# evandez/neuron-descriptions

Hardware: AMD Instinct MI355X
Metric: neuron-descriptions/sec (whole node), 4096 neurons x k=15 exemplars (higher is better)
Workload: dtype f32-equivalent: operands split into (hi,lo) f16 pairs (22 significant bits), 3 f16 MFMAs per product, f32 accumulate

## Files before the change

### neuron-descriptions_amd/csrc/common.h

```cpp
#pragma once
#include <hip/hip_runtime.h>
#include <stdint.h>
#include <stddef.h>
#include <string>
#include <vector>
#include <map>

#include "../../include/milan_hip.h"

#ifndef MILAN_EXPERIMENTS
#define MILAN_EXPERIMENTS 0
#endif

namespace milan {

void set_error(const char* fmt, ...);
#define MILAN_CHECK_HIP(expr)                                              \
  do {                                                                     \
    hipError_t _e = (expr);                                                \
    if (_e != hipSuccess) {                                                \
      milan::set_error("%s:%d: %s -> %s", __FILE__, __LINE__, #expr,       \
                       hipGetErrorString(_e));                             \
      return (int)_e;                                                      \
    }                                                                      \
// ... 54 lines not shown
  int chunk_major;
  float* C2;
  float* Cs;
  unsigned* status;
  int f16;
  const float* Wt;
  int tap_inner;
  const long long* lse_tgt;
  long lse_tgt_stride;
  float* lse_x;
  const int* m_live;
  const int* row_list;
  int m_live_mul;
  int tap_ncls;
  int tap_cls[MILAN_TAP_CLASSES][5];
};
static_assert(sizeof(GemmArgs) % 4 == 0, "GemmArgs is reloaded word by word");

enum OutMode : int { OUT_SCALAR = 0, OUT_VEC4 = 1, OUT_SPLIT8 = 2, OUT_F16 = 3 };

int launch_gemm(const GemmArgs& g, hipStream_t s);
bool row_list_supported(const GemmArgs& g);
void set_status_word(unsigned* word);
unsigned* status_word();
void profile_tag_kernel(int family);
int launch_zero_fill(void* p, size_t bytes, hipStream_t s);
int launch_f32_to_split(const float* src, long ld_src, float* dst, long ld_dst,
                        long rows, int K, float scale, hipStream_t s, int* nanrow = nullptr,
                        int stamp = 0);
int gemm_profile_enable(int enable);
int ensure_lds_attr(const void* kern, int bytes);
int device_cus8(int* out);
void* gemm_profile_begin(double flops, double bytes, hipStream_t s);
void gemm_profile_end(void* rec, hipStream_t s);

struct ShareArgs {
  const unsigned char* images;
// ... 410 lines not shown
```

### neuron-descriptions_amd/csrc/decoder.hip

```cpp
#include "common.h"
#include <limits>
#include <optional>

namespace milan {

static constexpr float kFloatMin = -3.402823466e+38f;

static const Tensor* find(milan_ctx* c, const std::string& name) {
  auto it = c->raw.find(name);
  return it == c->raw.end() ? nullptr : &it->second;
}

__global__ void pack_rows_kernel(const float* __restrict__ src, int n, int k,
                                 int kp, float* __restrict__ dst) {
  const long total = (long)n * kp;
  for (long idx = blockIdx.x * (long)blockDim.x + threadIdx.x; idx < total;
       idx += (long)gridDim.x * blockDim.x) {
    const int r = idx / kp, col = idx - (long)r * kp;
    dst[idx] = col < k ? src[(long)r * k + col] : 0.f;
  }
}

__device__ inline int lstm_source_row(int i, int hidden) {
  if (!hidden) return i;
// ... 157 lines not shown
    const int f = idx - i * F;
    float s = 0.f;
    for (int j = 0; j < k; ++j) {
      const float x = feat[(i * k + j) * F + f];
      sat = fmaxf(sat, fabsf(x * scale));
      s += x;
    }
    pooled[idx] = s / (float)k;
  }
  report_saturation(status, sat);
}

__global__ __launch_bounds__(256) void attend_kernel(
    const float* __restrict__ q, const float* __restrict__ keys,
    const float* __restrict__ w, const float* __restrict__ b, int rows, int rpn,
    int k, int A, float* __restrict__ att, const int* __restrict__ nanrow, int stamp) {
  const int r = blockIdx.x * 4 + (threadIdx.x >> 6);
  const int lane = threadIdx.x & 63;
  if (r >= rows) return;
  const float* qr = q + (long)r * A;
  const float* kr = keys + (long)(r / rpn) * k * A;
  float mine = 0.f;
  float mx = -INFINITY;
  for (int j = 0; j < k; ++j) {
    float s = 0.f;
    for (int a = lane; a < A; a += 64) s += w[a] * tanhf(qr[a] + kr[(long)j * A + a]);
    for (int o = 32; o > 0; o >>= 1) s += __shfl_xor(s, o);
    s += b[0];
    if (lane == (j & 63)) mine = s;
    mx = fmaxf(mx, s);
  }
  float e = lane < k ? expf(mine - mx) : 0.f;
  float sum = e;
  for (int o = 32; o > 0; o >>= 1) sum += __shfl_xor(sum, o);
  const bool bad = nanrow != nullptr && nanrow[r] == stamp;
  if (lane < k) att[(long)r * k + lane] = bad ? __builtin_nanf("") : e / sum;
}

constexpr int kAttMaxK = 16, kAttMaxE = 8;
__device__ __forceinline__ float tanh_exp2(float x) {
  const float t = __builtin_amdgcn_exp2f(x * 2.8853900817779268f);
  return 1.f - 2.f * __builtin_amdgcn_rcpf(t + 1.f);
}
__global__ __launch_bounds__(256) void attend16_kernel(
    const float* __restrict__ q, const float* __restrict__ keys,
    const float* __restrict__ w, const float* __restrict__ b, int rows, int rpn,
    int k, int A, float* __restrict__ att, const int* __restrict__ nanrow, int stamp) {
  const int neuron = blockIdx.x;
  const int wave = blockIdx.y * 4 + (threadIdx.x >> 6), lane = threadIdx.x & 63;
  const int stride = 4 * gridDim.y;
  const int r0 = neuron * rpn;
  const int r1 = r0 + rpn < rows ? r0 + rpn : rows;
  if (r0 + wave >= r1) return;
  const float* kr = keys + (long)neuron * k * A;
  const int ne = (A + 63) / 64;
  float wv[kAttMaxE], kv[kAttMaxK][kAttMaxE];
  int av[kAttMaxE];
#pragma unroll
  for (int e = 0; e < kAttMaxE; ++e) {
    const int a = lane + 64 * e;
    const bool ok = a < A;
    av[e] = ok ? a : 0;
    wv[e] = ok ? w[a] : 0.f;
  }
#pragma unroll
  for (int j = 0; j < kAttMaxK; ++j)
#pragma unroll
// ... 33 lines not shown
    float mx = valid ? s : -INFINITY;
#pragma unroll
    for (int X = 4; X < 64; X <<= 1) mx = fmaxf(mx, __shfl_xor(mx, X));
    const bool writer = valid && (lane & 3) == 0;
    const float ev = writer ? expf(s - mx) : 0.f;
    float sum = ev;
#pragma unroll
    for (int X = 4; X < 64; X <<= 1) sum += __shfl_xor(sum, X);
    const bool bad = nanrow != nullptr && nanrow[r] == stamp;
    if (writer) att[(long)r * k + j] = bad ? __builtin_nanf("") : ev / sum;
  }
}

static void launch_attend(const float* q, const float* keys, const float* w, const float* b,
                          int rows, int rpn, int k, int A, float* att, const int* nanrow,
                          int stamp, hipStream_t s) {
  static const bool fast = !(getenv("MILAN_ATTEND_FAST") && atoi(getenv("MILAN_ATTEND_FAST")) == 0);
  if (fast && k <= kAttMaxK && A <= 64 * kAttMaxE) {
    const int neurons = (rows + rpn - 1) / rpn;
    int rs = (4096 + neurons * 4 - 1) / (neurons * 4);
    const int rs_max = (rpn + 3) / 4;
    rs = rs < 1 ? 1 : (rs > rs_max ? rs_max : rs);
    hipLaunchKernelGGL(attend16_kernel, dim3(neurons, rs), dim3(256), 0, s, q, keys, w, b, rows,
                       rpn, k, A, att, nanrow, stamp);
  } else {
    hipLaunchKernelGGL(attend_kernel, dim3((rows + 3) / 4), dim3(256), 0, s, q, keys, w, b,
                       rows, rpn, k, A, att, nanrow, stamp);
  }
}

constexpr int kCtxMaxK = 16;
template <bool RESIDENT>
__global__ __launch_bounds__(256) void context_kernel(
    const float* __restrict__ att, const float* __restrict__ feat, int rows,
    int rpn, int k, int F, float* __restrict__ ctx, float scale,
    int* __restrict__ nanrow, int stamp) {
  const int neuron = blockIdx.x;
  const int f = (blockIdx.y * 256 + threadIdx.x) * 4;
  if (f >= F) return;
  const float* fr = feat + (long)neuron * k * F + f;
  float4 v[RESIDENT ? kCtxMaxK : 1];
  if constexpr (RESIDENT) {
#pragma unroll
    for (int j = 0; j < kCtxMaxK; ++j)
      v[j] = j < k ? *reinterpret_cast<const float4*>(fr + (long)j * F)
                   : make_float4(0.f, 0.f, 0.f, 0.f);
  }
  const int r0 = neuron * rpn;
  const int r1 = r0 + rpn < rows ? r0 + rpn : rows;
  for (int r = r0; r < r1; ++r) {
    const float* ar = att + (long)r * k;
    float s0 = 0.f, s1 = 0.f, s2 = 0.f, s3 = 0.f;
    if constexpr (RESIDENT) {
#pragma unroll
      for (int j = 0; j < kCtxMaxK; ++j) {
        if (j < k) {
          const float aj = ar[j];
          s0 = fmaf(aj, v[j].x, s0); s1 = fmaf(aj, v[j].y, s1);
          s2 = fmaf(aj, v[j].z, s2); s3 = fmaf(aj, v[j].w, s3);
        }
      }
    } else {
      for (int j = 0; j < k; ++j) {
        const float4 w = *reinterpret_cast<const float4*>(fr + (long)j * F);
// ... 17 lines not shown
                             float* __restrict__ dst, int ldd, float scale) {
  const long total = (long)rows * E;
  for (long idx = blockIdx.x * (long)blockDim.x + threadIdx.x; idx < total;
       idx += (long)gridDim.x * blockDim.x) {
    const long r = idx / E;
    const int e = idx - r * E;
    dst[r * ldd + e] = table[tok[r] * E + e] * scale;
  }
}

__global__ void embed_split_kernel(const float* __restrict__ table,
                                   const int64_t* __restrict__ tok, int rows, int E,
                                   float* __restrict__ dst, int ldd, float scale,
                                   unsigned* status,
                                   const int* __restrict__ live = nullptr,
                                   const int* __restrict__ nanrow = nullptr, int stamp = 0) {
  if (live) rows = min(rows, *live);
  const int g8 = E >> 3;
  const long total = (long)rows * g8;
  float sat = 0.f;
  for (long idx = blockIdx.x * (long)blockDim.x + threadIdx.x; idx < total;
       idx += (long)gridDim.x * blockDim.x) {
    const long r = idx / g8;
    const int q = idx - r * g8;
    const float* sp = table + tok[r] * E + q * 8;
    _Float16 hi[8], lo[8];
#pragma unroll
    for (int e = 0; e < 8; ++e) {
      const float x = fminf(fmaxf(sp[e] * scale, -65504.f), 65504.f);
      sat = fmaxf(sat, fabsf(x));
      hi[e] = (_Float16)x;
      lo[e] = (_Float16)(x - (float)hi[e]);
    }
    if (nanrow != nullptr && nanrow[r] == stamp) {
#pragma unroll
      for (int e = 0; e < 8; ++e) hi[e] = (_Float16)__builtin_nanf("");
    }
    float4* d = reinterpret_cast<float4*>(dst + r * ldd + q * 8);
    d[0] = *reinterpret_cast<const float4*>(hi);
    d[1] = *reinterpret_cast<const float4*>(lo);
  }
  report_saturation(status, sat);
}

__global__ void lstm_pointwise_kernel(const float* __restrict__ gates,
                                      const float* __restrict__ c_in, int rows,
                                      int H, float* __restrict__ h_out,
                                      float* __restrict__ c_out) {
  const long total = (long)rows * H;
// ... 580 lines not shown
  }
}

__global__ void beam_reorder_kernel(
    const int* __restrict__ new_tok, const int* __restrict__ new_bp, int n,
    int beam_prev, int beam, int H, const float* __restrict__ h_src,
    const float* __restrict__ c_src, float* __restrict__ h_dst,
    float* __restrict__ c_dst, int lm_layers, int Hl, long lm_rows_src,
    long lm_rows_dst, const float* __restrict__ hl_src,
    const float* __restrict__ cl_src, float* __restrict__ hl_dst,
    float* __restrict__ cl_dst, int64_t* __restrict__ tok_dst,
    int* __restrict__ hist_tok, int* __restrict__ hist_bp) {
  const int r = blockIdx.x;
  const int nn = r / beam;
  const int src = nn * beam_prev + new_bp[r];
  for (int j = threadIdx.x; j < H; j += blockDim.x) {
    h_dst[(long)r * H + j] = h_src[(long)src * H + j];
    c_dst[(long)r * H + j] = c_src[(long)src * H + j];
  }
  for (int l = 0; l < lm_layers; ++l)
    for (int j = threadIdx.x; j < Hl; j += blockDim.x) {
      hl_dst[((long)l * lm_rows_dst + r) * Hl + j] =
          hl_src[((long)l * lm_rows_src + src) * Hl + j];
      cl_dst[((long)l * lm_rows_dst + r) * Hl + j] =
          cl_src[((long)l * lm_rows_src + src) * Hl + j];
    }
  if (threadIdx.x == 0) {
    tok_dst[r] = new_tok[r];
    hist_tok[r] = new_tok[r];
    hist_bp[r] = new_bp[r];
  }
}

__global__ void beam_finalize_kernel(const int* __restrict__ hist_tok,
                                     const int* __restrict__ hist_bp, int n,
                                     int beam, int T,
                                     int64_t* __restrict__ beam_tokens) {
  const int r = blockIdx.x * blockDim.x + threadIdx.x;
  if (r >= n * beam) return;
  const int nn = r / beam;
  int j = r - nn * beam;
  const long R = (long)n * beam;
  for (int t = T - 1; t >= 0; --t) {
    beam_tokens[(long)r * T + t] = hist_tok[t * R + nn * beam + j];
    j = hist_bp[t * R + nn * beam + j];
  }
// ... 256 lines not shown

struct DecBuf {
  float *keys, *pooled, *x, *h, *cc, *hn, *cn, *q, *att, *ctx, *gates, *logits;
  float *lm_logits, *lm_emb, *lm_gates;
  LmState lm[2];
  float* cand_v; int* cand_i;
  float* last_lp[2]; int *new_tok, *new_bp, *hist_tok, *hist_bp;
  int64_t *tok, *seqs;
  float *lm_alive, *lm_total;
  float* lm_dedup; size_t lm_dedup_floats;
  int32_t* len1;
  float* scratch;
  size_t scratch_floats;
  int* nanrow;
  int nan_stamp;
};

static size_t lm_dedup_floats(const milan_dims& d, size_t R, int L, int G);

static void dec_plan(const milan_ctx* c, int n, int k, int beam, int T, bool lm,
                     Arena& a, DecBuf* b) {
  const milan_dims& d = c->d;
  const size_t R = (size_t)n * beam;
  const int F = d.feature_size, H = d.hidden_size, E = d.embedding_size,
            A = d.attention_size, V = d.vocab_size;
  b->keys = a.get<float>((size_t)n * k * A);
  b->pooled = a.get<float>((size_t)n * F);
  b->x = a.get<float>(R * (E + F));
  b->h = a.get<float>(R * H); b->cc = a.get<float>(R * H);
  b->hn = a.get<float>(R * H); b->cn = a.get<float>(R * H);
  b->q = a.get<float>(R * A);
  b->att = a.get<float>(R * k);
  b->ctx = a.get<float>(R * F);
  b->gates = a.get<float>(R * 4 * H);
  b->logits = a.get<float>(R * V);
  b->cand_v = a.get<float>(R * beam); b->cand_i = a.get<int>(R * beam);
  b->last_lp[0] = a.get<float>(R); b->last_lp[1] = a.get<float>(R);
  b->new_tok = a.get<int>(R); b->new_bp = a.get<int>(R);
  b->hist_tok = a.get<int>(R * T); b->hist_bp = a.get<int>(R * T);
  b->tok = a.get<int64_t>(R);
  b->seqs = a.get<int64_t>(R * (T + 1));
  b->len1 = a.get<int32_t>(2 * (size_t)n + 2);
  b->nanrow = a.get<int>(R);
  b->nan_stamp = 0;
  {
    const size_t rows = R > (size_t)n * k ? R : (size_t)n * k;
    b->scratch_floats = rows * (size_t)(E + F + d.hidden_size);
    b->scratch = a.get<float>(b->scratch_floats);
  }
  b->lm_logits = nullptr;
  b->lm_dedup = nullptr; b->lm_dedup_floats = 0;
  if (lm) {
    const int Hl = d.lm_hidden_size, El = d.lm_embedding_size;
    b->lm_logits = a.get<float>(R * V);
    b->lm_emb = a.get<float>(R * El);
    b->lm_gates = a.get<float>(R * 4 * Hl);
    for (int i = 0; i < 2; ++i) {
      b->lm[i].h = a.get<float>(R * Hl * d.lm_layers);
      b->lm[i].c = a.get<float>(R * Hl * d.lm_layers);
// ... 45 lines not shown
  return 0;
}

int decoder_init_state(milan_ctx* c, const float* features, int n, int k,
                       float* h, float* cc, Arena& ws, hipStream_t s) {
  MILAN_TRY(check_dims(c, k));
  float* pooled = ws.get<float>((size_t)n * c->d.feature_size);
  MILAN_REQUIRE(pooled, MILAN_ERR_WORKSPACE, "init_state: workspace too small");
  c->scratch_floats = (size_t)n * c->d.feature_size;
  c->scratch = ws.get<float>(c->scratch_floats);
  return init_state_impl(c, features, n, k, pooled, h, cc, s);
}

static void launch_context(const float* att, const float* features, int rows,
                           int rpn, int k, int F, float* ctx, float scale,
                           int* nanrow, int stamp, hipStream_t s) {
  const int gy = (F / 4 + 255) / 256;
  const int neurons = (rows + rpn - 1) / rpn;
  if (k <= kCtxMaxK)
    hipLaunchKernelGGL(context_kernel<true>, dim3(neurons, gy), dim3(256), 0, s,
                       att, features, rows, rpn, k, F, ctx, scale, nanrow, stamp);
  else
    hipLaunchKernelGGL(context_kernel<false>, dim3(neurons, gy), dim3(256), 0, s,
                       att, features, rows, rpn, k, F, ctx, scale, nanrow, stamp);
}

static int step_core(milan_ctx* c, const float* features, const float* keys,
                     int rows, int rpn, int k, const int64_t* tok,
                     const float* h, const float* cc, float* hn, float* cn,
                     DecBuf* b, hipStream_t s) {
  const milan_dims& d = c->d;
  const int F = d.feature_size, H = d.hidden_size, E = d.embedding_size,
            A = d.attention_size, V = d.vocab_size;
  const int ldx = E + F;
  const bool fused = c->precision == MILAN_PRECISION_SPLIT_F16 && c->scratch &&
                     c->q2h.ws && c->gate.ws && c->lstm_cat.ws && c->out.ws &&
                     E % 16 == 0 && F % 8 == 0 && H % 16 == 0 &&
                     (size_t)rows * (ldx + H) <= c->scratch_floats;
  const bool cat_split = c->precision == MILAN_PRECISION_SPLIT_F16 && c->lstm_cat.ws &&
                         c->scratch && (size_t)rows * c->lstm_cat.k <= c->scratch_floats;
  const float fs = cat_split ? c->feat_scale : 1.f;
  if (fused) {
    float* xs = c->scratch;
    float* hs = c->scratch + (size_t)rows * ldx;
    float* hs2 = b->gates;
    const int stamp = ++b->nan_stamp;
    MILAN_TRY(launch_f32_to_split(h, H, hs, H, rows, H, 1.f, s, b->nanrow, stamp));
    auto split_lin = [&](const LinearW& w, float* C, int ldc, int epi,
                         const float* aux, int ldaux) {
      GemmArgs g = linear_args(hs, H, w.ws, w.b, C, ldc, rows, w.n, w.k, epi,
                               c->zero, aux, ldaux);
      g.a_split = 1;
      g.acc_scale = w.ws_inv;
      return g;
    };
    MILAN_TRY(launch_gemm(split_lin(c->q2h, b->q, A, EPI_BIAS, nullptr, 0), s));
// ... 554 lines not shown
                "row select: rows=%d, k=%d must be in 1..min(%d, vocab_size %d)", rows, k,
                kMaxBeam, V);
  if (path == 0)
    return launch_row_select(logits, lm_logits, lambda, rows, V, k, last_tok, stop,
                             cand_v, cand_i, nullptr, 0, s);
  if (path == 1)
    return launch_row_select_wide(logits, lm_logits, lambda, rows, V, k, last_tok, stop,
                                  cand_v, cand_i, s);
  MILAN_REQUIRE(k >= 2 && row_select_reg_ok(V, k), MILAN_ERR_ARG,
                "row select: path %d needs 2 <= k <= 256 and vocab_size <= %d (k=%d, "
                "vocab_size %d)", path, kRowRegs * 256, k, V);
  return launch_row_select(logits, lm_logits, lambda, rows, V, k, last_tok, stop, cand_v,
                           cand_i, nullptr, 0, s, false, path == 2 ? 0 : 2);
}

int decoder_decode(milan_ctx* c, const float* features, int n, int k,
                   int strategy, int length, int beam, int mi, float temperature,
                   int group_size, int64_t* tokens, float* scores,
                   float* predictions, float* attentions, int64_t* beam_tokens,
                   float* beam_scores, int32_t* out_len, Arena& ws,
                   hipStream_t s) {
  MILAN_TRY(check_dims(c, k));
  const milan_dims& d = c->d;
  const int H = d.hidden_size, V = d.vocab_size;
  MILAN_REQUIRE(strategy == MILAN_GREEDY || strategy == MILAN_FORCED ||
                    strategy == MILAN_BEAM || strategy == MILAN_RERANK,
                MILAN_ERR_ARG, "unknown strategy: %d", strategy);
  MILAN_REQUIRE(!(mi && strategy == MILAN_RERANK), MILAN_ERR_ARG,
                "cannot set `mi=` decoding when reranking");
  MILAN_REQUIRE(!(mi || strategy == MILAN_RERANK) || d.has_lm, MILAN_ERR_NO_LM,
// ... 68 lines not shown
                           predictions + (long)t * V, (long)length * V, V, b.att,
                           n, k, t, length, tokens, scores, attentions, b.tok);
      else
        hipLaunchKernelGGL(greedy_record_kernel, dim3(nblk_all(n)), dim3(256), 0, s,
                           b.cand_v, b.cand_i, b.att, n, k, t, length, tokens,
                           scores, attentions, b.tok);
      float* tmp = h; h = hn; hn = tmp;
      tmp = cc; cc = cn; cn = tmp;
    }
    MILAN_CHECK_HIP(hipGetLastError());
    return 0;
  }

  const bool wide = c->beam_path == 1;
  int beam_prev = 1, rows = n, lpcur = 0;
  std::optional<StageScope> search_scope;
  search_scope.emplace(MILAN_STAGE_DEC_SEARCH, s);
  for (int t = 0; t < length; ++t) {
    MILAN_TRY(step_core(c, features, b.keys, rows, beam_prev, k, b.tok, b.h, b.cc,
                        b.hn, b.cn, &b, s));
    const float* lm_logits = nullptr;
    if (mi) {
      b.lm[lmcur].rows = b.lm[lmcur ^ 1].rows = R;
      MILAN_TRY(lm_step(c, b.tok, rows, b.lm[lmcur], b.lm[lmcur ^ 1], b.lm_emb,
                        b.lm_gates, b.lm_logits, s));
      lm_logits = b.lm_logits;
    }
    MILAN_TRY(launch_row_select(b.logits, lm_logits, temperature, rows, V, beam,
                                t == 0 ? nullptr : b.tok, d.stop_index, b.cand_v,
                                b.cand_i, nullptr, 0, s, wide));
    MILAN_TRY(decoder_beam_merge(b.cand_v, b.cand_i, t == 0 ? nullptr : b.last_lp[lpcur],
                                 n, beam_prev, beam, wide, b.last_lp[lpcur ^ 1], b.new_tok,
                                 b.new_bp, s));
    lpcur ^= 1;
    hipLaunchKernelGGL(
        beam_reorder_kernel, dim3(R), dim3(128), 0, s, b.new_tok, b.new_bp, n,
        beam_prev, beam, H, b.hn, b.cn, b.h, b.cc, mi ? d.lm_layers : 0, Hl,
        (long)R, (long)R, mi ? b.lm[lmcur ^ 1].h : nullptr,
        mi ? b.lm[lmcur ^ 1].c : nullptr, mi ? b.lm[lmcur].h : nullptr,
        mi ? b.lm[lmcur].c : nullptr, b.tok, b.hist_tok + (long)t * R,
        b.hist_bp + (long)t * R);
    beam_prev = beam;
    rows = R;
  }
  hipLaunchKernelGGL(beam_finalize_kernel, dim3(nblk_all(R)), dim3(256), 0, s,
                     b.hist_tok, b.hist_bp, n, beam, length, beam_tokens);
  MILAN_CHECK_HIP(hipMemcpyAsync(beam_scores, b.last_lp[lpcur],
                                 sizeof(float) * R, hipMemcpyDeviceToDevice, s));
  const int groups = (n + group_size - 1) / group_size;
  int32_t* lens = out_len ? out_len : b.len1 + n + 1;
  hipLaunchKernelGGL(group_len_kernel, dim3(groups), dim3(256), 0, s, b.hist_tok,
                     n, beam, length, group_size, d.stop_index, lens);
// ... 23 lines not shown
```

### neuron-descriptions_amd/csrc/gemm.hip

```cpp
#include "common.h"

#include <map>
#include <mutex>
#include <utility>

#include <cstdio>
#include <cstdlib>
#include <cstring>
#include <type_traits>
#include <utility>
#include <vector>

#ifndef MILAN_ABLATE_BUILD
#define MILAN_ABLATE_BUILD 0
#endif
#ifndef MILAN_EXPERIMENTS
#define MILAN_EXPERIMENTS 0
#endif

namespace milan {

typedef float f32x16 __attribute__((ext_vector_type(16)));
typedef float f32x4 __attribute__((ext_vector_type(4)));
typedef _Float16 f16x8 __attribute__((ext_vector_type(8)));
// ... 1482 lines not shown
    if (cls < 0 && b < first + B) { cls = c; cfirst = first; ctiles = T; }
    first += B;
  }
  if (cls < 0) return false;
  const int bl = b - cfirst;
  if ((bl >> 3) >= (ctiles >> 3) + ((bl & 7) < (ctiles & 7))) return false;
  const int tile = xcd_tile(bl, ctiles);
  t->j = tile / tiles_n;
  t->tile_n = tile - t->j * tiles_n;
  t->y0 = cw[cls * 5]; t->ny = cw[cls * 5 + 1]; t->x0 = cw[cls * 5 + 2]; t->nx = cw[cls * 5 + 3];
  t->mask = (unsigned)cw[cls * 5 + 4];
  t->cnt = imgs * t->ny * t->nx;
  return true;
}

template <int BNW, bool F16 = false, bool TAPI = false, bool LIST = false>
__device__ __forceinline__ void split16_pp32_tile(int tile_m, int tile_n, int tid, bool prefetched,
                                                  bool has_next, int ntile_m, int ntile_n,
                                                  TapTile tt = TapTile{}) {
  const GemmArgs g = reload_gemm_args();
  constexpr int BM = 256, BN = 256, BKP = 32, TM = BNW == 256 ? 4 : 2, TN = 2;
  static_assert(BNW == 256 || BNW == 128, "ping-pong tile: 256 or 128 columns");
  constexpr int SLOTF = BM * BKP;
  constexpr unsigned OOB = 0x80000000u;
  extern __shared__ __attribute__((aligned(16))) float smem[];
  auto a_slot = [&](int sl) { return smem + (sl < 2 ? sl : 3) * SLOTF; };
  auto w_slot = [&](int sl) { return smem + (sl == 0 ? 2 : 4) * SLOTF; };
  const int lane = tid & 63;
  const int wave = __builtin_amdgcn_readfirstlane(tid >> 6);
  const int wm = BNW == 256 ? wave >> 2 : wave >> 1, wn = BNW == 256 ? wave & 3 : wave & 1;
  const int group = wave >> 2;
// ... 40 lines not shown
    ho += ((ho + 1) * pix_row <= rem);
    *dimg_out = dimg;
    *wo_out = rem - ho * pix_row + (TAPI ? tt.x0 : 0);
    *ho_out = ho + (TAPI ? tt.y0 : 0);
    return ok;
  };
  auto setup = [&](PpLoader& L, int tm, int tn) {
    const int prow = lane >> 3, pos = lane & 7;
    const int m0 = tm * BM;
    const int img0 = LIST ? list_slot0(m0) : m0 / pix_img;
    const int rem0 = LIST ? img0 * pix_img : m0 - img0 * pix_img;
    const long bias = ((long)g.pad * g.Wd + g.pad) * g.a_pix_stride;
    L.srd_a = __builtin_amdgcn_make_buffer_rsrc(
        const_cast<float*>(g.A + (long)img0 * g.a_img_stride - bias), 0, 0x7fffffff, 0x00020000);
    L.srd_a2 = __builtin_amdgcn_make_buffer_rsrc(
        const_cast<float*>(g.A2 ? g.A2 + (long)img0 * g.a2_img_stride : g.A), 0, 0x7fffffff,
        0x00020000);
    L.srd_w = __builtin_amdgcn_make_buffer_rsrc(const_cast<float*>(g.W + (long)tn * BNW * g.Kp), 0,
                                                0x7fffffff, 0x00020000);
#pragma unroll
    for (int it = 0; it < 4; ++it) {
      const int row = it * 64 + wave * 8 + prow;
      const int q = pos ^ ((row >> 1) & 7);
      int dimg, ho, wo;
      const bool ok = row_pixel(m0, rem0, row, &dimg, &ho, &wo);
      const int hi0 = ho * g.stride - g.pad, wi0 = wo * g.stride - g.pad;
      L.hw0[it] = (hi0 << 16) | (wi0 & 0xffff);
      if constexpr (TAPI) {
        unsigned m = 0;
        for (int kh = 0, t = 0; kh < g.KH; ++kh)
          for (int kw = 0; kw < g.KW; ++kw, ++t)
            m |= (unsigned)((unsigned)(hi0 + kh) < (unsigned)g.H &&
                            (unsigned)(wi0 + kw) < (unsigned)g.Wd) << t;
        L.mask[it] = m;
      }
      L.row_off[it] = ok ? (unsigned)(((long)dimg * g.a_img_stride +
                                       ((long)hi0 * g.Wd + wi0) * g.a_pix_stride + bias + q * 4) * 4)
                         : OOB;
      L.row_off2[it] = (ok && g.A2)
                           ? (unsigned)(((long)dimg * g.a2_img_stride +
                                         ((long)(ho * g.stride2) * g.W2d + wo * g.stride2) *
                                             g.a2_pix_stride + q * 4) * 4)
                           : OOB;
      L.vb[it] = (row < BNW && tn * BNW + row < g.N) ? (unsigned)(((long)row * g.Kp + q * 4) * 4) : OOB;
    }
    L.ia = L.iw = L.is_kh = L.is_kw = L.is_cin0 = 0;
    L.a_bits = L.w_bits = tt.mask;
    L.w_slice = 0;
    L.cin_limit = g.Cin;
    L.cur_srd = L.srd_a;
    set_tap(L);
  };
  auto issue_a = [&](PpLoader& L, auto slot_tag, bool really) {
    constexpr int SLOT = decltype(slot_tag)::value;
    if (really) {
      int woff = wave * (8 * BKP);
      asm volatile("" : "+s"(woff));
      float* dst = a_slot(SLOT) + woff;
// ... 322 lines not shown
  const int q = blockIdx.x;
  if (q >= T) return;
  const int tile = xcd_tile(q, T);
  const int tile_m = tile / tiles_n, tile_n = tile - tile_m * tiles_n;
  TapTile tt{};
  if constexpr (TAPI) {
    tt.ny = g.Ho; tt.nx = g.Wo;
    tt.mask = 0xffffffffu >> (32 - g.KH * g.KW);
    tt.cnt = g.M;
  }
  int tid = threadIdx.x;
  asm volatile("" : "+v"(tid));
  split16_pp32_tile<256, false, TAPI, true>(tile_m, tile_n, tid, false, false, tile_m, tile_n, tt);
}

template <int BNW, bool TAPI>
__global__ __launch_bounds__(512, 2) void igemm_f16_pp32_kernel(GemmArgs g, int tiles_m, int tiles_n) {
  tiles_m = live_tiles_m(g, tiles_m, 256);
  if constexpr (TAPI) {
    TapTile tt;
    if (!tap_tile(g, tiles_m, tiles_n, &tt)) return;
    int tid = threadIdx.x;
    asm volatile("" : "+v"(tid));
    split16_pp32_tile<BNW, true, true>(tt.j, tt.tile_n, tid, false, false, tt.j, tt.tile_n, tt);
  } else {
    const int T = tiles_m * tiles_n;
    const int q = blockIdx.x;
    if (q >= T) return;
    const int tile = xcd_tile(q, T);
    const int tile_m = tile / tiles_n, tile_n = tile - tile_m * tiles_n;
// ... 548 lines not shown
      memcpy(cls[at], c, sizeof(c));
      if (ry[a].n * rx[b].n < min_pix) min_pix = ry[a].n * rx[b].n;
    }
  if ((256L / min_pix + 2) * t.a_img_stride * 4 + 64 >= 0x7fffffffL) return tiles_m * tiles_n;
  const long imgs = t.M / howo;
  long grid = 0;
  for (int c = 0; c < n; ++c)
    grid += ((imgs * cls[c][1] * cls[c][3] + 255) / 256 * tiles_n + 7) / 8 * 8;
  if (grid >= 0x7fffffffL) return tiles_m * tiles_n;
  t.tap_ncls = n;
  memcpy(t.tap_cls, cls, sizeof(int) * 5 * n);
  return (int)grid;
}

static thread_local bool t_row_list_taken = false;

template <int BNW>
static int launch_split16_pp32(const GemmArgs& g, hipStream_t s) {
  const int tiles_m = (g.M + 255) / 256, tiles_n = (g.N + BNW - 1) / BNW;
  const size_t lds = size_t(5) * 256 * 32 * sizeof(float);
  if (g.row_list != nullptr) {
    if (BNW != 256) return MILAN_ERR_SHAPE;
    t_row_list_taken = true;
    GemmArgs t = g;
    const bool tapi = tap_inner_wanted(g);
    if (tapi) { t.W = g.Wt; t.tap_inner = 1; }
    t.tap_ncls = 0;
    profile_tag_kernel(tapi ? MILAN_KERNEL_PP32T_256 : MILAN_KERNEL_PP32_256);
    auto kern = tapi ? igemm_split16_pp32l_kernel<true> : igemm_split16_pp32l_kernel<false>;
    MILAN_TRY(ensure_lds_attr(reinterpret_cast<const void*>(kern), (int)lds));
    hipLaunchKernelGGL(kern, dim3(tiles_m * tiles_n), dim3(512), lds, s, t, tiles_m, tiles_n);
    MILAN_CHECK_HIP(hipGetLastError());
    return 0;
  }
  if (tap_inner_wanted(g)) {
    GemmArgs t = g;
    t.W = g.Wt;
    t.tap_inner = 1;
    const int grid = tap_classes(t, tiles_m, tiles_n);
    profile_tag_kernel(BNW == 256 ? MILAN_KERNEL_PP32T_256 : MILAN_KERNEL_PP32_128);
    auto kern = igemm_split16_pp32t_kernel<BNW>;
    MILAN_TRY(ensure_lds_attr(reinterpret_cast<const void*>(kern), (int)lds));
    hipLaunchKernelGGL(kern, dim3(grid), dim3(512), lds, s, t, tiles_m, tiles_n);
    MILAN_CHECK_HIP(hipGetLastError());
    return 0;
  }
// ... 174 lines not shown
  if (!g.a_split || g.f16 || g.chunk_major || g.aniso || g.tile_hint != 0 || env_tile_hint() != 0 ||
      env_tile_override(g.N, g.K) != 0 || pp != 1)
    return false;
#if MILAN_EXPERIMENTS
  if (conv3x3_enabled() || (getenv("MILAN_SCHED") && atoi(getenv("MILAN_SCHED")))) return false;
#endif
  if (g.epilogue == EPI_LSE || g.epilogue == EPI_LSTM || !g.out_split) return false;
  if (g.N % 256 != 0 || g.Cin % 32 != 0 || g.K != g.Kp || !pp_eligible(g)) return false;
  if (g.A2 && (g.K1 % 32 != 0 || g.KH != 1 || g.KW != 1)) return false;
  if (g.KH * g.KW > 1 && !tap_inner_wanted(g)) return false;
  if ((long)g.H + g.pad >= 32768 || (long)g.Wd + g.pad >= 32768) return false;
  if (howo <= 0 || g.M % howo != 0 || 257 * howo >= (1L << 24)) return false;
  if (258 * g.a_img_stride * 4 + 64 >= 0x7fffffffL) return false;
  if (g.A2 && 258 * g.a2_img_stride * 4 + 64 >= 0x7fffffffL) return false;
  return true;
}

static int launch_gemm_impl(GemmArgs g, hipStream_t s) {
  const bool cin32 = (g.Cin % 32 == 0);
  if (g.status == nullptr) g.status = status_word();
  if (g.tile_hint == 0) g.tile_hint = env_tile_hint();
  if (const int o = env_tile_override(g.N, g.K)) g.tile_hint = o;
  {
    static int dbg = -1;
    if (dbg < 0) { const char* e = getenv("MILAN_ABLATE"); dbg = e ? atoi(e) : 0; }
    g.debug = dbg;
#if MILAN_EXPERIMENTS
    static int stg = -1;
    if (stg < 0) { const char* e = getenv("MILAN_STAGGER"); stg = e ? atoi(e) : 0; }
    static int stg_all = -1;
// ... 110 lines not shown
               : launch_cfg<128, 128, 2, false, false>(g, s);
}

static int launch_gemm_checked(const GemmArgs& g, hipStream_t s);
int launch_gemm(const GemmArgs& g, hipStream_t s) {
  MILAN_REQUIRE(g.M > 0 && g.N > 0 && g.K > 0, MILAN_ERR_SHAPE,
                "gemm: empty problem M=%d N=%d K=%d", g.M, g.N, g.K);
  MILAN_REQUIRE(g.row_list == nullptr || row_list_supported(g), MILAN_ERR_SHAPE,
                "gemm: no row-list form of this launch (N=%d Cin=%d %dx%d)", g.N, g.Cin, g.KH, g.KW);
  MILAN_REQUIRE(g.Cin % 4 == 0 && g.a_pix_stride % 4 == 0 &&
                    g.a_img_stride % 4 == 0 && g.Kp % 32 == 0 && aligned16(g.A) &&
                    aligned16(g.W),
                MILAN_ERR_SHAPE,
                "gemm: Cin=%d / strides must be multiples of 4 floats and "
                "operands 16-byte aligned", g.Cin);
  if (g.row_list != nullptr) {
    t_row_list_taken = false;
    const int r = launch_gemm_checked(g, s);
    MILAN_REQUIRE(r != 0 || t_row_list_taken, MILAN_ERR_STATE,
                  "gemm: a row-list launch was dispatched to a kernel without a list form "
                  "(row_list_supported() no longer matches the dispatch)");
    return r;
  }
  return launch_gemm_checked(g, s);
}

static int launch_gemm_checked(const GemmArgs& g, hipStream_t s) {
  if (!g_prof.on) return launch_gemm_impl(g, s);
  ProfRec* e = prof_next();
  MILAN_REQUIRE(e != nullptr, MILAN_ERR_STATE, "profiler: cannot create events");
// ... 15 lines not shown
```

Measured before the change: 1425.

## Share parent-dependent decoder work across beams with identical back-pointers

During beam search, rows whose back-pointer names the same parent have identical hidden states for the attention query, attention, context and gate computations. New kernels build per-neuron parent classes (dedup, scan, fill), and the step runs q2h, attention, context and gate only on the unique parent rows. The LSTM GEMM then gathers its second operand through a row table (new A2TAB kernel variant), and the reorder kernel skips copying h. This cuts redundant GEMM and attention work when beams share parents, at the cost of extra small launches and an indirect row load in the GEMM.

Result: no change. 1437 (median of 5 runs) (+0.8%).

```diff
diff --git a/neuron-descriptions_amd/csrc/common.h b/neuron-descriptions_amd/csrc/common.h
--- a/neuron-descriptions_amd/csrc/common.h
+++ b/neuron-descriptions_amd/csrc/common.h
@@ -92,6 +92,7 @@
   int m_live_mul;
   int tap_ncls;
   int tap_cls[MILAN_TAP_CLASSES][5];
+  const int* a2_rows;
 };
 static_assert(sizeof(GemmArgs) % 4 == 0, "GemmArgs is reloaded word by word");
 
@@ -99,6 +100,7 @@
 
 int launch_gemm(const GemmArgs& g, hipStream_t s);
 bool row_list_supported(const GemmArgs& g);
+bool a2_rows_supported(const GemmArgs& g);
 void set_status_word(unsigned* word);
 unsigned* status_word();
 void profile_tag_kernel(int family);
diff --git a/neuron-descriptions_amd/csrc/decoder.hip b/neuron-descriptions_amd/csrc/decoder.hip
--- a/neuron-descriptions_amd/csrc/decoder.hip
+++ b/neuron-descriptions_amd/csrc/decoder.hip
@@ -195,12 +195,14 @@
 __global__ __launch_bounds__(256) void attend_kernel(
     const float* __restrict__ q, const float* __restrict__ keys,
     const float* __restrict__ w, const float* __restrict__ b, int rows, int rpn,
-    int k, int A, float* __restrict__ att, const int* __restrict__ nanrow, int stamp) {
+    int k, int A, float* __restrict__ att, const int* __restrict__ nanrow, int stamp,
+    const int* __restrict__ rep = nullptr, const int* __restrict__ live = nullptr) {
   const int r = blockIdx.x * 4 + (threadIdx.x >> 6);
   const int lane = threadIdx.x & 63;
+  if (live) rows = min(rows, *live);
   if (r >= rows) return;
   const float* qr = q + (long)r * A;
-  const float* kr = keys + (long)(r / rpn) * k * A;
+  const float* kr = keys + (long)((rep ? rep[r] : r) / rpn) * k * A;
   float mine = 0.f;
   float mx = -INFINITY;
   for (int j = 0; j < k; ++j) {
@@ -226,12 +228,13 @@
 __global__ __launch_bounds__(256) void attend16_kernel(
     const float* __restrict__ q, const float* __restrict__ keys,
     const float* __restrict__ w, const float* __restrict__ b, int rows, int rpn,
-    int k, int A, float* __restrict__ att, const int* __restrict__ nanrow, int stamp) {
+    int k, int A, float* __restrict__ att, const int* __restrict__ nanrow, int stamp,
+    const int* __restrict__ coff = nullptr) {
   const int neuron = blockIdx.x;
   const int wave = blockIdx.y * 4 + (threadIdx.x >> 6), lane = threadIdx.x & 63;
   const int stride = 4 * gridDim.y;
-  const int r0 = neuron * rpn;
-  const int r1 = r0 + rpn < rows ? r0 + rpn : rows;
+  const int r0 = coff ? coff[neuron] : neuron * rpn;
+  const int r1 = coff ? coff[neuron + 1] : r0 + rpn < rows ? r0 + rpn : rows;
   if (r0 + wave >= r1) return;
   const float* kr = keys + (long)neuron * k * A;
   const int ne = (A + 63) / 64;
@@ -295,7 +298,8 @@
 
 static void launch_attend(const float* q, const float* keys, const float* w, const float* b,
                           int rows, int rpn, int k, int A, float* att, const int* nanrow,
-                          int stamp, hipStream_t s) {
+                          int stamp, hipStream_t s, const int* coff = nullptr,
+                          const int* rep = nullptr, int rpn_src = 0) {
   static const bool fast = !(getenv("MILAN_ATTEND_FAST") && atoi(getenv("MILAN_ATTEND_FAST")) == 0);
   if (fast && k <= kAttMaxK && A <= 64 * kAttMaxE) {
     const int neurons = (rows + rpn - 1) / rpn;
@@ -303,7 +307,10 @@
     const int rs_max = (rpn + 3) / 4;
     rs = rs < 1 ? 1 : (rs > rs_max ? rs_max : rs);
     hipLaunchKernelGGL(attend16_kernel, dim3(neurons, rs), dim3(256), 0, s, q, keys, w, b, rows,
-                       rpn, k, A, att, nanrow, stamp);
+                       rpn, k, A, att, nanrow, stamp, coff);
+  } else if (coff) {
+    hipLaunchKernelGGL(attend_kernel, dim3((rows + 3) / 4), dim3(256), 0, s, q, keys, w, b,
+                       rows, rpn_src, k, A, att, nanrow, stamp, rep, coff + (rows + rpn - 1) / rpn);
   } else {
     hipLaunchKernelGGL(attend_kernel, dim3((rows + 3) / 4), dim3(256), 0, s, q, keys, w, b,
                        rows, rpn, k, A, att, nanrow, stamp);
@@ -315,7 +322,7 @@
 __global__ __launch_bounds__(256) void context_kernel(
     const float* __restrict__ att, const float* __restrict__ feat, int rows,
     int rpn, int k, int F, float* __restrict__ ctx, float scale,
-    int* __restrict__ nanrow, int stamp) {
+    int* __restrict__ nanrow, int stamp, const int* __restrict__ coff = nullptr) {
   const int neuron = blockIdx.x;
   const int f = (blockIdx.y * 256 + threadIdx.x) * 4;
   if (f >= F) return;
@@ -327,8 +334,8 @@
       v[j] = j < k ? *reinterpret_cast<const float4*>(fr + (long)j * F)
                    : make_float4(0.f, 0.f, 0.f, 0.f);
   }
-  const int r0 = neuron * rpn;
-  const int r1 = r0 + rpn < rows ? r0 + rpn : rows;
+  const int r0 = coff ? coff[neuron] : neuron * rpn;
+  const int r1 = coff ? coff[neuron + 1] : r0 + rpn < rows ? r0 + rpn : rows;
   for (int r = r0; r < r1; ++r) {
     const float* ar = att + (long)r * k;
     float s0 = 0.f, s1 = 0.f, s2 = 0.f, s3 = 0.f;
@@ -376,7 +383,8 @@
                                    float* __restrict__ dst, int ldd, float scale,
                                    unsigned* status,
                                    const int* __restrict__ live = nullptr,
-                                   const int* __restrict__ nanrow = nullptr, int stamp = 0) {
+                                   const int* __restrict__ nanrow = nullptr, int stamp = 0,
+                                   const int* __restrict__ cls = nullptr) {
   if (live) rows = min(rows, *live);
   const int g8 = E >> 3;
   const long total = (long)rows * g8;
@@ -394,7 +402,7 @@
       hi[e] = (_Float16)x;
       lo[e] = (_Float16)(x - (float)hi[e]);
     }
-    if (nanrow != nullptr && nanrow[r] == stamp) {
+    if (nanrow != nullptr && nanrow[cls ? cls[r] : r] == stamp) {
 #pragma unroll
       for (int e = 0; e < 8; ++e) hi[e] = (_Float16)__builtin_nanf("");
     }
@@ -1005,9 +1013,14 @@
   const int r = blockIdx.x;
   const int nn = r / beam;
   const int src = nn * beam_prev + new_bp[r];
-  for (int j = threadIdx.x; j < H; j += blockDim.x) {
-    h_dst[(long)r * H + j] = h_src[(long)src * H + j];
-    c_dst[(long)r * H + j] = c_src[(long)src * H + j];
+  if (h_dst != nullptr) {
+    for (int j = threadIdx.x; j < H; j += blockDim.x) {
+      h_dst[(long)r * H + j] = h_src[(long)src * H + j];
+      c_dst[(long)r * H + j] = c_src[(long)src * H + j];
+    }
+  } else {
+    for (int j = threadIdx.x; j < H; j += blockDim.x)
+      c_dst[(long)r * H + j] = c_src[(long)src * H + j];
   }
   for (int l = 0; l < lm_layers; ++l)
     for (int j = threadIdx.x; j < Hl; j += blockDim.x) {
@@ -1021,6 +1034,106 @@
     hist_tok[r] = new_tok[r];
     hist_bp[r] = new_bp[r];
   }
+}
+
+__global__ __launch_bounds__(64) void beam_class_kernel(
+    const int* __restrict__ new_bp, int beam_prev, int beam, int* __restrict__ cls,
+    int* __restrict__ rep_local, int* __restrict__ cnt) {
+  __shared__ unsigned present[32];
+  __shared__ int base[33];
+  const int n = blockIdx.x, lane = threadIdx.x;
+  if (lane < 32) present[lane] = 0u;
+  __syncthreads();
+  for (int j = lane; j < beam; j += 64) {
+    const int bp = new_bp[(long)n * beam + j];
+    atomicOr(&present[(bp >> 5) & 31], 1u << (bp & 31));
+  }
+  __syncthreads();
+  if (lane == 0) {
+    int acc = 0;
+    for (int w = 0; w < 32; ++w) { base[w] = acc; acc += __popc(present[w]); }
+    base[32] = acc;
+    cnt[n] = acc;
+  }
+  __syncthreads();
+  auto rank = [&](int v) {
+    const int w = (v >> 5) & 31;
+    return base[w] + __popc(present[w] & ((1u << (v & 31)) - 1u));
+  };
+  for (int j = lane; j < beam; j += 64) cls[(long)n * beam + j] = rank(new_bp[(long)n * beam + j]);
+  for (int v = lane; v < beam_prev; v += 64)
+    if ((present[v >> 5] >> (v & 31)) & 1u) rep_local[(long)n * beam + rank(v)] = n * beam_prev + v;
+}
+
+__global__ __launch_bounds__(1024) void beam_class_scan_kernel(const int* __restrict__ cnt, int n,
+                                                               int* __restrict__ off) {
+  __shared__ int wsum[16];
+  __shared__ int carry;
+  const int tid = threadIdx.x, lane = tid & 63, wave = tid >> 6;
+  if (tid == 0) { carry = 0; off[0] = 0; }
+  __syncthreads();
+  for (int i0 = 0; i0 < n; i0 += 1024) {
+    const int i = i0 + tid;
+    int v = i < n ? cnt[i] : 0;
+    for (int o = 1; o < 64; o <<= 1) {
+      const int u = __shfl_up(v, o);
+      if (lane >= o) v += u;
+    }
+    if (lane == 63) wsum[wave] = v;
+    __syncthreads();
+    int before = carry;
+    for (int w = 0; w < wave; ++w) before += wsum[w];
+    if (i < n) off[i + 1] = before + v;
+    __syncthreads();
+    if (tid == 1023) carry = before + v;
+    __syncthreads();
+  }
+}
+
+__global__ void beam_class_fill_kernel(const int* __restrict__ off, const int* __restrict__ cnt,
+                                       const int* __restrict__ rep_local, int rows, int beam,
+                                       int* __restrict__ cls, int* __restrict__ rep) {
+  const int r = blockIdx.x * blockDim.x + threadIdx.x;
+  if (r >= rows) return;
+  const int n = r / beam, j = r - n * beam;
+  const int o = off[n];
+  cls[r] += o;
+  if (j < cnt[n]) rep[o + j] = rep_local[r];
+}
+
+__global__ void class_split_kernel(const float* __restrict__ h, int H,
+                                   const int* __restrict__ rep, const int* __restrict__ live,
+                                   int rows, float* __restrict__ dst, long ldd,
+                                   unsigned* status, int* __restrict__ nanrow, int stamp) {
+  typedef float v4f __attribute__((ext_vector_type(4)));
+  rows = min(rows, *live);
+  const int g8 = H >> 3;
+  const long total = (long)rows * g8;
+  float sat = 0.f;
+  for (long idx = blockIdx.x * (long)blockDim.x + threadIdx.x; idx < total;
+       idx += (long)gridDim.x * blockDim.x) {
+    const long u = idx / g8;
+    const int q = idx - u * g8;
+    const float* sp = h + (long)rep[u] * H + q * 8;
+    const v4f a = *reinterpret_cast<const v4f*>(sp);
+    const v4f b = *reinterpret_cast<const v4f*>(sp + 4);
+    float v[8];
+#pragma unroll
+    for (int e = 0; e < 4; ++e) { v[e] = a[e]; v[4 + e] = b[e]; }
+    bool bad = false;
+#pragma unroll
+    for (int e = 0; e < 8; ++e) {
+      bad |= v[e] != v[e];
+      v[e] = v[e] != v[e] ? 0.f : v[e];
+    }
+    if (bad) nanrow[u] = stamp;
+    v4f hi, lo;
+    split8_rne(v, &hi, &lo, &sat);
+    float* d = dst + u * ldd + q * 8;
+    *reinterpret_cast<v4f*>(d) = hi;
+    *reinterpret_cast<v4f*>(d + 4) = lo;
+  }
+  report_saturation(status, sat);
 }
 
 __global__ void beam_finalize_kernel(const int* __restrict__ hist_tok,
@@ -1307,6 +1420,13 @@
   size_t scratch_floats;
   int* nanrow;
   int nan_stamp;
+  int *cls, *crep, *crep_local, *ccnt, *coff;
+};
+
+struct BeamShare {
+  const int *cls, *rep, *coff;
+  const int* live;
+  int rpn_src;
 };
 
 static size_t lm_dedup_floats(const milan_dims& d, size_t R, int L, int G);
@@ -1336,6 +1456,8 @@
   b->len1 = a.get<int32_t>(2 * (size_t)n + 2);
   b->nanrow = a.get<int>(R);
   b->nan_stamp = 0;
+  b->cls = a.get<int>(R); b->crep = a.get<int>(R); b->crep_local = a.get<int>(R);
+  b->ccnt = a.get<int>((size_t)n); b->coff = a.get<int>((size_t)n + 1);
   {
     const size_t rows = R > (size_t)n * k ? R : (size_t)n * k;
     b->scratch_floats = rows * (size_t)(E + F + d.hidden_size);
@@ -1411,21 +1533,21 @@
 
 static void launch_context(const float* att, const float* features, int rows,
                            int rpn, int k, int F, float* ctx, float scale,
-                           int* nanrow, int stamp, hipStream_t s) {
+                           int* nanrow, int stamp, hipStream_t s, const int* coff = nullptr) {
   const int gy = (F / 4 + 255) / 256;
   const int neurons = (rows + rpn - 1) / rpn;
   if (k <= kCtxMaxK)
     hipLaunchKernelGGL(context_kernel<true>, dim3(neurons, gy), dim3(256), 0, s,
-                       att, features, rows, rpn, k, F, ctx, scale, nanrow, stamp);
+                       att, features, rows, rpn, k, F, ctx, scale, nanrow, stamp, coff);
   else
     hipLaunchKernelGGL(context_kernel<false>, dim3(neurons, gy), dim3(256), 0, s,
-                       att, features, rows, rpn, k, F, ctx, scale, nanrow, stamp);
+                       att, features, rows, rpn, k, F, ctx, scale, nanrow, stamp, coff);
 }
 
 static int step_core(milan_ctx* c, const float* features, const float* keys,
                      int rows, int rpn, int k, const int64_t* tok,
                      const float* h, const float* cc, float* hn, float* cn,
-                     DecBuf* b, hipStream_t s) {
+                     DecBuf* b, hipStream_t s, const BeamShare* sh = nullptr) {
   const milan_dims& d = c->d;
   const int F = d.feature_size, H = d.hidden_size, E = d.embedding_size,
             A = d.attention_size, V = d.vocab_size;
@@ -1437,6 +1559,61 @@
   const bool cat_split = c->precision == MILAN_PRECISION_SPLIT_F16 && c->lstm_cat.ws &&
                          c->scratch && (size_t)rows * c->lstm_cat.k <= c->scratch_floats;
   const float fs = cat_split ? c->feat_scale : 1.f;
+  MILAN_REQUIRE(sh == nullptr || fused, MILAN_ERR_STATE,
+                "decoder step: parent classes need the fused split-f16 branch");
+  if (fused && sh != nullptr) {
+    const int ldc = F + H;
+    float* es = c->scratch;
+    float* cb = c->scratch + (size_t)rows * E;
+    float* hs2 = b->gates;
+    const int stamp = ++b->nan_stamp;
+    {
+      long blocks = ((long)rows * (H >> 3) + 255) / 256;
+      blocks = blocks > 16384 ? 16384 : blocks;
+      hipLaunchKernelGGL(class_split_kernel, dim3((int)blocks), dim3(256), 0, s, h, H, sh->rep,
+                         sh->live, rows, cb + F, (long)ldc, status_word(), b->nanrow, stamp);
+    }
+    auto class_lin = [&](const LinearW& w, float* C, int ldcc, int epi, const float* aux,
+                         int ldaux) {
+      GemmArgs g = linear_args(cb + F, ldc, w.ws, w.b, C, ldcc, rows, w.n, w.k, epi, c->zero,
+                               aux, ldaux);
+      g.a_split = 1;
+      g.acc_scale = w.ws_inv;
+      g.m_live = sh->live; g.m_live_mul = 1;
+      return g;
+    };
+    MILAN_TRY(launch_gemm(class_lin(c->q2h, b->q, A, EPI_BIAS, nullptr, 0), s));
+    launch_attend(b->q, keys, c->att_w, c->att_b, rows, rpn, k, A, b->att, b->nanrow, stamp, s,
+                  sh->coff, sh->rep, sh->rpn_src);
+    launch_context(b->att, features, rows, rpn, k, F, b->ctx, fs, b->nanrow, stamp, s, sh->coff);
+    {
+      GemmArgs g = class_lin(c->gate, cb, ldc, EPI_BIAS_SIGMUL, b->ctx, F);
+      g.out_split = 1;
+      MILAN_TRY(launch_gemm(g, s));
+    }
+    hipLaunchKernelGGL(embed_split_kernel, dim3(nblk((long)rows * (E / 8))),
+                       dim3(256), 0, s, c->embedding, tok, rows, E, es, E, c->emb_scale,
+                       status_word(), nullptr, b->nanrow, stamp, sh->cls);
+    {
+      const LinearW& w = c->lstm_cat;
+      GemmArgs g = linear_args(es, E, w.ws, w.b, hn, H, rows, w.n, w.k, EPI_LSTM, c->zero, cc, H);
+      g.C2 = cn; g.Cs = hs2;
+      g.a_split = 1;
+      g.acc_scale = w.ws_inv;
+      g.Cin = E;
+      g.A2 = cb; g.K1 = E; g.H2 = 1; g.W2d = 1; g.stride2 = 1;
+      g.a2_pix_stride = ldc; g.a2_img_stride = ldc;
+      g.a2_rows = sh->cls;
+      MILAN_TRY(launch_gemm(g, s));
+    }
+    GemmArgs g = linear_args(hs2, H, c->out.ws, c->out.b, b->logits, V, rows, c->out.n, c->out.k,
+                             EPI_BIAS, c->zero);
+    g.a_split = 1;
+    g.acc_scale = c->out.ws_inv;
+    MILAN_TRY(launch_gemm(g, s));
+    MILAN_CHECK_HIP(hipGetLastError());
+    return 0;
+  }
   if (fused) {
     float* xs = c->scratch;
     float* hs = c->scratch + (size_t)rows * ldx;
@@ -2021,6 +2198,40 @@
                            cand_i, nullptr, 0, s, false, path == 2 ? 0 : 2);
 }
 
+static int beam_share_mode() {
+  static const int mode = getenv("MILAN_BEAM_SHARE") ? atoi(getenv("MILAN_BEAM_SHARE")) : 1;
+  return mode;
+}
+static bool share_ok(const milan_ctx* c, int R, int beam) {
+  const bool on = beam_share_mode() != 0;
+  const milan_dims& d = c->d;
+  const int F = d.feature_size, H = d.hidden_size, E = d.embedding_size;
+  if (!on || beam < 2 || beam > kMaxBeam) return false;
+  const bool fused = c->precision == MILAN_PRECISION_SPLIT_F16 && c->scratch && c->q2h.ws &&
+                     c->gate.ws && c->lstm_cat.ws && c->out.ws && E % 16 == 0 && F % 8 == 0 &&
+                     H % 16 == 0 && (size_t)R * (E + F + H) <= c->scratch_floats;
+  if (!fused || !c->lstm_cat.gate_interleaved) return false;
+  const LinearW& w = c->lstm_cat;
+  GemmArgs g = linear_args(c->scratch, E, w.ws, w.b, nullptr, H, R, w.n, w.k, EPI_LSTM, c->zero);
+  g.a_split = 1;
+  g.Cin = E;
+  g.A2 = c->scratch; g.K1 = E; g.H2 = 1; g.W2d = 1; g.stride2 = 1;
+  g.a2_pix_stride = F + H; g.a2_img_stride = F + H;
+  g.a2_rows = reinterpret_cast<const int*>(c->scratch);
+  return a2_rows_supported(g);
+}
+
+static int launch_beam_classes(DecBuf* b, int n, int beam_prev, int beam, hipStream_t s) {
+  const int R = n * beam;
+  hipLaunchKernelGGL(beam_class_kernel, dim3(n), dim3(64), 0, s, b->new_bp, beam_prev, beam,
+                     b->cls, b->crep_local, b->ccnt);
+  hipLaunchKernelGGL(beam_class_scan_kernel, dim3(1), dim3(1024), 0, s, b->ccnt, n, b->coff);
+  hipLaunchKernelGGL(beam_class_fill_kernel, dim3(nblk_all(R)), dim3(256), 0, s, b->coff,
+                     b->ccnt, b->crep_local, R, beam, b->cls, b->crep);
+  MILAN_CHECK_HIP(hipGetLastError());
+  return 0;
+}
+
 int decoder_decode(milan_ctx* c, const float* features, int n, int k,
                    int strategy, int length, int beam, int mi, float temperature,
                    int group_size, int64_t* tokens, float* scores,
@@ -2119,11 +2330,20 @@
 
   const bool wide = c->beam_path == 1;
   int beam_prev = 1, rows = n, lpcur = 0;
+  const bool share = share_ok(c, R, beam);
+  MILAN_REQUIRE(share || beam_share_mode() != 2 || beam < 2, MILAN_ERR_STATE,
+                "decode: MILAN_BEAM_SHARE=2, but this beam search cannot share its parents' "
+                "work (needs the fused split-f16 step and embedding_size %% 32 == 0)");
+  BeamShare sh{b.cls, b.crep, b.coff, b.coff + n, 1};
   std::optional<StageScope> search_scope;
   search_scope.emplace(MILAN_STAGE_DEC_SEARCH, s);
   for (int t = 0; t < length; ++t) {
-    MILAN_TRY(step_core(c, features, b.keys, rows, beam_prev, k, b.tok, b.h, b.cc,
-                        b.hn, b.cn, &b, s));
+    if (share && t > 0)
+      MILAN_TRY(step_core(c, features, b.keys, rows, beam_prev, k, b.tok, b.hn, b.cc,
+                          b.hn, b.cn, &b, s, &sh));
+    else
+      MILAN_TRY(step_core(c, features, b.keys, rows, beam_prev, k, b.tok, b.h, b.cc,
+                          b.hn, b.cn, &b, s));
     const float* lm_logits = nullptr;
     if (mi) {
       b.lm[lmcur].rows = b.lm[lmcur ^ 1].rows = R;
@@ -2138,9 +2358,13 @@
                                  n, beam_prev, beam, wide, b.last_lp[lpcur ^ 1], b.new_tok,
                                  b.new_bp, s));
     lpcur ^= 1;
+    if (share && t + 1 < length) {
+      MILAN_TRY(launch_beam_classes(&b, n, beam_prev, beam, s));
+      sh.rpn_src = beam_prev;
+    }
     hipLaunchKernelGGL(
         beam_reorder_kernel, dim3(R), dim3(128), 0, s, b.new_tok, b.new_bp, n,
-        beam_prev, beam, H, b.hn, b.cn, b.h, b.cc, mi ? d.lm_layers : 0, Hl,
+        beam_prev, beam, H, b.hn, b.cn, share ? nullptr : b.h, b.cc, mi ? d.lm_layers : 0, Hl,
         (long)R, (long)R, mi ? b.lm[lmcur ^ 1].h : nullptr,
         mi ? b.lm[lmcur ^ 1].c : nullptr, mi ? b.lm[lmcur].h : nullptr,
         mi ? b.lm[lmcur].c : nullptr, b.tok, b.hist_tok + (long)t * R,
diff --git a/neuron-descriptions_amd/csrc/gemm.hip b/neuron-descriptions_amd/csrc/gemm.hip
--- a/neuron-descriptions_amd/csrc/gemm.hip
+++ b/neuron-descriptions_amd/csrc/gemm.hip
@@ -1520,7 +1520,7 @@
   return true;
 }
 
-template <int BNW, bool F16 = false, bool TAPI = false, bool LIST = false>
+template <int BNW, bool F16 = false, bool TAPI = false, bool LIST = false, bool A2TAB = false>
 __device__ __forceinline__ void split16_pp32_tile(int tile_m, int tile_n, int tid, bool prefetched,
                                                   bool has_next, int ntile_m, int ntile_n,
                                                   TapTile tt = TapTile{}) {
@@ -1591,8 +1591,8 @@
     L.srd_a = __builtin_amdgcn_make_buffer_rsrc(
         const_cast<float*>(g.A + (long)img0 * g.a_img_stride - bias), 0, 0x7fffffff, 0x00020000);
     L.srd_a2 = __builtin_amdgcn_make_buffer_rsrc(
-        const_cast<float*>(g.A2 ? g.A2 + (long)img0 * g.a2_img_stride : g.A), 0, 0x7fffffff,
-        0x00020000);
+        const_cast<float*>(A2TAB ? g.A2 : g.A2 ? g.A2 + (long)img0 * g.a2_img_stride : g.A), 0,
+        0x7fffffff, 0x00020000);
     L.srd_w = __builtin_amdgcn_make_buffer_rsrc(const_cast<float*>(g.W + (long)tn * BNW * g.Kp), 0,
                                                 0x7fffffff, 0x00020000);
 #pragma unroll
@@ -1614,11 +1614,17 @@
       L.row_off[it] = ok ? (unsigned)(((long)dimg * g.a_img_stride +
                                        ((long)hi0 * g.Wd + wi0) * g.a_pix_stride + bias + q * 4) * 4)
                          : OOB;
-      L.row_off2[it] = (ok && g.A2)
-                           ? (unsigned)(((long)dimg * g.a2_img_stride +
-                                         ((long)(ho * g.stride2) * g.W2d + wo * g.stride2) *
-                                             g.a2_pix_stride + q * 4) * 4)
-                           : OOB;
+      if constexpr (A2TAB) {
+        const int src = g.a2_rows[m0 + (ok ? row : 0)];
+        L.row_off2[it] = ok ? (unsigned)(((long)src * g.a2_img_stride + q * 4) * 4) : OOB;
+        asm volatile("" : "+v"(L.row_off2[it]));
+      } else {
+        L.row_off2[it] = (ok && g.A2)
+                             ? (unsigned)(((long)dimg * g.a2_img_stride +
+                                           ((long)(ho * g.stride2) * g.W2d + wo * g.stride2) *
+                                               g.a2_pix_stride + q * 4) * 4)
+                             : OOB;
+      }
       L.vb[it] = (row < BNW && tn * BNW + row < g.N) ? (unsigned)(((long)row * g.Kp + q * 4) * 4) : OOB;
     }
     L.ia = L.iw = L.is_kh = L.is_kw = L.is_cin0 = 0;
@@ -1971,6 +1977,21 @@
   split16_pp32_tile<256, false, TAPI, true>(tile_m, tile_n, tid, false, false, tile_m, tile_n, tt);
 }
 
+template <int BNW>
+__global__ __launch_bounds__(512, 2) void igemm_split16_pp32r_kernel(GemmArgs g, int tiles_m,
+                                                                     int tiles_n) {
+  tiles_m = live_tiles_m(g, tiles_m, 256);
+  const int T = tiles_m * tiles_n;
+  const int q = blockIdx.x;
+  if (q >= T) return;
+  const int tile = xcd_tile(q, T);
+  const int tile_m = tile / tiles_n, tile_n = tile - tile_m * tiles_n;
+  int tid = threadIdx.x;
+  asm volatile("" : "+v"(tid));
+  split16_pp32_tile<BNW, false, false, false, true>(tile_m, tile_n, tid, false, false, tile_m,
+                                                    tile_n);
+}
+
 template <int BNW, bool TAPI>
 __global__ __launch_bounds__(512, 2) void igemm_f16_pp32_kernel(GemmArgs g, int tiles_m, int tiles_n) {
   tiles_m = live_tiles_m(g, tiles_m, 256);
@@ -2549,6 +2570,7 @@
 }
 
 static thread_local bool t_row_list_taken = false;
+static thread_local bool t_a2_rows_taken = false;
 
 template <int BNW>
 static int launch_split16_pp32(const GemmArgs& g, hipStream_t s) {
@@ -2565,6 +2587,15 @@
     auto kern = tapi ? igemm_split16_pp32l_kernel<true> : igemm_split16_pp32l_kernel<false>;
     MILAN_TRY(ensure_lds_attr(reinterpret_cast<const void*>(kern), (int)lds));
     hipLaunchKernelGGL(kern, dim3(tiles_m * tiles_n), dim3(512), lds, s, t, tiles_m, tiles_n);
+    MILAN_CHECK_HIP(hipGetLastError());
+    return 0;
+  }
+  if (g.a2_rows != nullptr) {
+    t_a2_rows_taken = true;
+    profile_tag_kernel(BNW == 256 ? MILAN_KERNEL_PP32_256 : MILAN_KERNEL_PP32_128);
+    auto kern = igemm_split16_pp32r_kernel<BNW>;
+    MILAN_TRY(ensure_lds_attr(reinterpret_cast<const void*>(kern), (int)lds));
+    hipLaunchKernelGGL(kern, dim3(tiles_m * tiles_n), dim3(512), lds, s, g, tiles_m, tiles_n);
     MILAN_CHECK_HIP(hipGetLastError());
     return 0;
   }
@@ -2769,6 +2800,24 @@
   if (258 * g.a_img_stride * 4 + 64 >= 0x7fffffffL) return false;
   if (g.A2 && 258 * g.a2_img_stride * 4 + 64 >= 0x7fffffffL) return false;
   return true;
+}
+
+bool a2_rows_supported(const GemmArgs& g) {
+  static int pp = -1, pp128 = -1;
+  if (pp < 0) { const char* e = getenv("MILAN_PP"); pp = e ? atoi(e) : 1; }
+  if (pp128 < 0) { const char* e = getenv("MILAN_PP128"); pp128 = e ? atoi(e) : 1; }
+  if (g.a2_rows == nullptr || g.A2 == nullptr || g.row_list != nullptr) return false;
+  if (!g.a_split || g.f16 || g.chunk_major || g.aniso || g.tile_hint != 0 || env_tile_hint() != 0 ||
+      env_tile_override(g.N, g.K) != 0)
+    return false;
+  if (g.KH != 1 || g.KW != 1 || g.pad != 0 || g.stride != 1 || g.H != 1 || g.Wd != 1 ||
+      g.Ho != 1 || g.Wo != 1 || g.H2 != 1 || g.W2d != 1 || g.stride2 != 1)
+    return false;
+  if (g.N <= 64 || g.Cin % 32 != 0 || g.K1 % 32 != 0 || g.K1 <= 0 || !pp_eligible(g)) return false;
+  const int pad256 = (g.N + 255) / 256 * 256 - g.N, pad128 = (g.N + 127) / 128 * 128 - g.N;
+  const bool wide = g.N % 256 == 0 || (g.N > 2048 && pad256 <= pad128);
+  if (wide ? pp != 1 : pp128 == 0) return false;
+  return (long)g.M * g.a2_img_stride * 4 + 64 < 0x7fffffffL;
 }
 
 static int launch_gemm_impl(GemmArgs g, hipStream_t s) {
@@ -2909,6 +2958,16 @@
                 MILAN_ERR_SHAPE,
                 "gemm: Cin=%d / strides must be multiples of 4 floats and "
                 "operands 16-byte aligned", g.Cin);
+  MILAN_REQUIRE(g.a2_rows == nullptr || a2_rows_supported(g), MILAN_ERR_SHAPE,
+                "gemm: no row-table form of this launch (N=%d Cin=%d K1=%d)", g.N, g.Cin, g.K1);
+  if (g.a2_rows != nullptr) {
+    t_a2_rows_taken = false;
+    const int r = launch_gemm_checked(g, s);
+    MILAN_REQUIRE(r != 0 || t_a2_rows_taken, MILAN_ERR_STATE,
+                  "gemm: a row-table launch was dispatched to a kernel without a table form "
+                  "(a2_rows_supported() no longer matches the dispatch)");
+    return r;
+  }
   if (g.row_list != nullptr) {
     t_row_list_taken = false;
     const int r = launch_gemm_checked(g, s);
```
